# Shinokawa/Fast-SCNN-pytorch

Measured on AMD Instinct MI355X. Metric: images/sec fwd+bwd @1024x2048 bs=8 per GPU; 1/2/4/8-GPU scaling, higher is better.
Workload: dtype bf16; 1 GPU; cfg3 train step: fwd + CE(ignore -1) + bwd + fused SGD (fused low-res upsample+CE head); model=FastSCNN (19 classes), global_batch=8, per_gpu_batch=8, parallelism=dp1

## Files before the change

fast-scnn-pytorch_amd/_lib.py:

```python
import ctypes
import os
import threading

_HERE = os.path.dirname(os.path.abspath(__file__))
LIB_PATH = os.environ.get("FSCNN_LIB", os.path.join(_HERE, "libfastscnn_hip.so"))

DT_F32, DT_BF16, DT_F16 = 0, 1, 2
DT_U8 = 3

c_int, c_ll, c_float, c_vp, c_char_p = (ctypes.c_int, ctypes.c_longlong, ctypes.c_float,
                                        ctypes.c_void_p, ctypes.c_char_p)
c_ull, c_double = ctypes.c_ulonglong, ctypes.c_double
P_int, P_ll, P_vp = ctypes.POINTER(c_int), ctypes.POINTER(c_ll), ctypes.POINTER(c_vp)
P_float = ctypes.POINTER(c_float)
P_double = ctypes.POINTER(c_double)
c_uint, P_ubyte = ctypes.c_uint, ctypes.POINTER(ctypes.c_ubyte)


class AuxHead(ctypes.Structure):
    _fields_ = [("head", c_int), ("aux_weight", c_float), ("ignore_index", c_ll),
                ("smooth", c_float), ("dice_weight", c_float), ("focal_weight", c_float),
                ("alpha", c_float), ("gamma", c_float), ("thresh", c_float), ("min_kept", c_ll),
                ("class_weight", c_vp)]

# ... 110 lines not shown
                          c_int, c_float, c_vp]),
    "fscnn_adamw": (c_int, [c_vp, c_vp, c_vp, c_vp, c_vp, c_ll, c_double, c_double, c_double,
                            c_double, c_double, c_int, c_int, c_vp, c_int, c_vp, c_vp, c_vp]),
    "fscnn_adamw_segments": (c_int, [c_vp, c_vp, c_vp, c_vp, c_vp, c_vp, c_vp, c_int, c_vp, c_int,
                                     c_vp, c_int, c_vp, c_int, c_int, c_vp, c_vp, c_vp]),
    "fscnn_conv0_fwd": (c_int, [c_vp, c_int, c_int, c_int, c_int, c_vp, c_vp, c_vp, c_int, c_vp,
                                c_int, c_vp]),
    "fscnn_conv0_wgrad_slab_floats": (c_ll, [c_int, c_int, c_int]),
    "fscnn_conv0_wgrad": (c_int, [c_vp, c_int, c_int, c_int, c_int, c_vp, c_int, c_vp, c_vp, c_vp]),
    "fscnn_dw3x3_fwd": (c_int, [c_vp, c_int, c_int, c_int, c_int, c_int, c_int, c_vp, c_vp, c_vp,
                                c_int, c_vp, c_vp]),
    "fscnn_dw3x3_dgrad": (c_int, [c_vp, c_int, c_int, c_int, c_int, c_int, c_int, c_vp, c_vp,
                                  c_vp]),
    "fscnn_dw3x3_wgrad_slab_floats": (c_ll, [c_int, c_int, c_int, c_int, c_int, c_int]),
    "fscnn_dw3x3_wgrad": (c_int, [c_vp, c_vp, c_int, c_int, c_int, c_int, c_int, c_int, c_vp,
                                  c_vp, c_vp]),
    "fscnn_pw_gemm": (c_int, [c_int, c_int, c_int, c_vp, c_int, c_vp, c_int, c_int, c_vp, c_vp,
                              c_vp, c_int, c_int, c_vp, c_int, c_vp, c_int, c_vp]),
    "fscnn_pw_dgrad_bnbwd": (c_int, [c_int, c_int, c_int, c_vp, c_int, c_vp, c_int, c_vp, c_int,
                                     c_vp, c_int, c_vp, c_int, c_vp, c_vp, c_vp, c_vp, c_int,
                                     c_vp, c_vp, c_vp, c_vp, c_vp, c_vp, c_int, P_int, c_vp]),
    "fscnn_kth_smallest": (c_int, [c_vp, c_ll, c_ll, c_vp, c_vp, c_vp]),
    "fscnn_debug_stamps": (c_int, [c_vp, c_int]),
    "fscnn_debug_stamp_count": (c_int, []),
    "fscnn_debug_stamp_tag": (c_char_p, [c_int]),
    "fscnn_pw_wgrad_slab_floats": (c_ll, [c_int, c_int, c_int]),
    "fscnn_pw_gemm_stats_parts": (c_int, [c_int, c_int, c_int, c_int, c_int, c_int]),
    "fscnn_pw_wgrad": (c_int, [c_int, c_int, c_int, c_vp, c_int, c_vp, c_int, c_vp, c_vp, c_int,
                               c_vp]),
    "fscnn_bn_finalize": (c_int, [c_vp, c_int, c_int, c_vp, c_vp, c_vp, c_vp, c_vp, c_float,
                                  c_vp, c_vp, c_vp, c_vp, c_vp]),
    "fscnn_bilinear_ac_fwd": (c_int, [c_vp, c_int, c_int, c_int, c_int, c_int, c_int, c_int,
                                      c_vp, c_int, c_int, c_vp]),
    "fscnn_bilinear_ac_bwd": (c_int, [c_vp, c_int, c_int, c_int, c_int, c_int, c_int, c_int,
                                      c_vp, c_vp, c_vp]),
    "fscnn_pyramid_pool_fwd": (c_int, [c_vp, c_int, c_int, c_int, c_int, c_int, c_int, c_vp,
                                       c_vp]),
    "fscnn_block_ir_fwd": (c_int, [c_vp, c_int, c_int, c_int, c_int, c_int, c_int, c_int, c_int,
                                   c_vp, c_vp, c_vp, c_vp, c_vp, c_vp, c_vp, c_vp, c_vp, c_int,
                                   c_vp, c_int, c_vp]),
    "fscnn_pyramid_pool_bwd": (c_int, [c_vp, c_int, c_int, c_int, c_int, c_int, c_vp, c_int,
                                       c_int, c_vp]),
    "fscnn_bn_apply": (c_int, [c_ll, c_int, c_vp, c_int, c_vp, c_vp, c_vp, c_int, c_vp, c_vp, c_vp,
                               c_int, c_int, c_vp, c_int, c_int, c_vp]),
    "fscnn_bn_bwd": (c_int, [c_ll, c_int, c_vp, c_int, c_vp, c_int, c_vp, c_vp, c_vp, c_vp, c_vp,
                             c_int, c_int, c_vp, c_vp, c_vp, c_vp, c_vp, c_vp, c_vp, c_vp, c_vp,
                             c_vp, c_vp, c_vp, c_vp, c_int, P_int, P_int, c_vp]),
    "fscnn_ppm_branches_ok": (c_int, [c_int, c_int, c_int]),
    "fscnn_ppm_branches_fwd": (c_int, [c_int, P_int, c_int, c_vp, c_vp, c_vp, c_vp, c_vp, c_vp,
                                       c_vp, c_float, c_vp, c_vp, c_int, c_vp, c_vp, c_vp, c_vp,
                                       c_int, c_vp]),
    "fscnn_ppm_branches_bwd": (c_int, [c_int, P_int, c_int, c_vp, c_int, c_vp, c_int, c_vp, c_vp,
                                       c_vp, c_vp, c_vp, c_vp, c_vp, c_vp, c_vp, c_vp, c_vp, c_int,
                                       c_vp]),
    "fscnn_ppm_up_fwd": (c_int, [c_vp, c_int, c_int, c_int, c_int, c_vp, c_int, c_int, c_vp]),
    "fscnn_ppm_up_bwd": (c_int, [c_vp, c_int, c_int, c_int, c_int, c_int, c_int, c_vp, c_vp]),
    "fscnn_dropout": (c_int, [c_vp, c_int, c_int, c_int, c_int, c_int, c_int, c_ull, c_vp, c_ull,
                              c_float, c_vp, c_vp, c_vp, c_int, c_vp]),
    "fscnn_dw3x3_parts": (c_int, [c_int, c_int, c_int, c_int, c_int, c_int, c_int]),
    "fscnn_dw3x3_ct_width": (c_int, [c_int, c_int, c_int, c_int, c_int, c_int]),
    "fscnn_dw3x3_fwd_train": (c_int, [c_vp, c_int, c_int, c_int, c_int, c_int, c_int, c_vp, c_vp,
                                      c_vp, c_vp, c_vp, c_vp, c_vp, c_vp, c_vp, c_vp, c_vp, c_vp,
                                      c_float, c_vp, c_vp, c_vp, c_vp, P_int, c_vp]),
    "fscnn_dw3x3_dgrad_bn": (c_int, [c_vp, c_int, c_int, c_int, c_int, c_int, c_int, c_vp, c_vp,
                                     c_vp, c_vp, c_vp, c_vp, c_vp, c_int, c_vp, c_vp, c_vp, c_vp,
                                     c_vp, c_vp, P_int, c_vp]),
    "fscnn_dw3x3_wgrad_train": (c_int, [c_vp, c_vp, c_int, c_int, c_int, c_int, c_int, c_int,
                                        c_vp, c_vp, c_vp, c_vp, c_vp]),
    "fscnn_pw_fwd_train_route": (c_int, [c_int, c_int, c_int, c_int, c_int, c_int, c_int, P_int]),
    "fscnn_pw_fwd_train": (c_int, [c_int, c_int, c_int, c_vp, c_int, c_vp, c_vp, c_vp, c_int, c_vp,
                                   c_vp, c_int, c_vp, c_vp, c_vp, c_vp, c_vp, c_vp, c_vp, c_vp,
                                   c_float, c_vp, c_vp, c_vp, c_vp, c_int, P_int, P_int, c_vp]),
    "fscnn_pw_wgrad_train": (c_int, [c_int, c_int, c_int, c_vp, c_int, c_vp, c_int, c_vp, c_vp,
                                     c_vp, c_vp, c_vp, c_vp, c_int, P_int, c_vp]),
    "fscnn_pw_dgrad_train_route": (c_int, [c_int, c_int, c_int, c_int, c_int, c_int, c_int, c_int,
                                           P_int]),
    "fscnn_pw_dgrad_train": (c_int, [c_int, c_int, c_int, c_vp, c_int, c_vp, c_int, c_vp, c_int,
                                     c_vp, c_int, c_vp, c_int, c_vp, c_vp, c_vp, c_vp, c_int,
                                     c_vp, c_vp, c_vp, c_vp, c_vp, c_vp, c_vp, c_int, c_float,
                                     c_ull, c_ull, c_vp, c_int, P_int, P_int, c_vp]),
    "fscnn_im2col3": (c_int, [c_vp, c_int, c_int, c_int, c_int, c_int, c_int, c_vp, c_int, c_vp]),
    "fscnn_col2im3": (c_int, [c_vp, c_int, c_int, c_int, c_int, c_int, c_int, c_vp, c_int, c_int,
                              c_vp]),
    "fscnn_block_ir_s2_fwd": (c_int, [c_vp, c_int, c_int, c_int, c_int, c_int, c_int, c_int, c_int,
                                      c_vp, c_vp, c_vp, c_vp, c_vp, c_vp, c_vp, c_vp, c_vp, c_vp,
                                      c_int, c_vp]),
    "fscnn_block_ltd_fwd": (c_int, [c_vp, c_int, c_int, c_int, c_int, c_int, c_vp, c_vp, c_vp,
                                    c_vp, c_vp, c_vp, c_vp, c_vp, c_vp, c_vp, c_int, c_vp]),
    "fscnn_block_dsconv_fwd": (c_int, [c_vp, c_int, c_int, c_int, c_int, c_int, c_int, c_vp, c_vp,
                                       c_vp, c_vp, c_vp, c_vp, c_vp, c_int, c_vp]),
    "fscnn_block_dsconv_res_fwd": (c_int, [c_vp, c_int, c_int, c_int, c_int, c_int, c_int, c_int,
                                           c_int, c_vp, c_vp, c_vp, c_vp, c_vp, c_vp, c_vp, c_int,
                                           c_vp, c_int, c_vp]),
    "fscnn_block_cls_fwd": (c_int, [c_vp, c_int, c_int, c_int, c_int] + [c_vp] * 14 + [c_int, c_vp, c_vp,
                                                                              c_int, c_vp]),
    "fscnn_block_ffm_fwd": (c_int, [c_vp, c_int, c_int, c_int, c_int, c_int, c_int, c_vp, c_int,
                                    c_vp, c_vp, c_vp, c_vp, c_vp, c_vp, c_vp, c_vp, c_vp, c_vp,
                                    c_int, c_vp]),
}

_lib = None
_lock = threading.Lock()


def load():
    global _lib
    if _lib is not None:
        return _lib
    with _lock:
        if _lib is not None:
            return _lib
        if not os.path.exists(LIB_PATH):
            raise RuntimeError(
                "libfastscnn_hip.so not found at %s — build it with "
                "`python -c 'import __graft_entry__; __graft_entry__.build()'` "
                "(there is no CPU fallback)" % LIB_PATH)
        import torch
        lib = ctypes.CDLL(LIB_PATH, mode=ctypes.RTLD_GLOBAL)
        for name, (res, args) in SIGNATURES.items():
            fn = getattr(lib, name)
            fn.restype = res
            fn.argtypes = args
        _lib = lib
        return lib


def check(rc, what=""):
    if rc != 0:
        msg = load().fscnn_last_error().decode(errors="replace")
        raise RuntimeError("fastscnn HIP error %d in %s: %s" % (rc, what, msg))


def call(name, *args):
    rc = getattr(load(), name)(*args)
    check(rc, name)
    return rc


def ptr(t):
    return None if t is None else c_vp(t.data_ptr())


def stream_ptr(device=None):
    import torch
    return c_vp(torch.cuda.current_stream(device).cuda_stream)


def dtype_code(dt):
    import torch
    if dt == torch.float32:
        return DT_F32
    if dt == torch.bfloat16:
        return DT_BF16
    if dt == torch.float16:
        return DT_F16
    raise RuntimeError("fastscnn: unsupported dtype %s (fp32 / bf16 / fp16)" % (dt,))
```

fast-scnn-pytorch_amd/csrc/capi.cpp:

```cpp
#include <algorithm>
#include <chrono>
#include <cmath>
#include <cstdlib>
#include <cstdarg>
#include <cstdio>
#include <cstring>
#include <new>
#include <string>

#include "../../include/fastscnn.h"
#include "net.hpp"

namespace fscnn {

static thread_local char g_err[512] = "";

void set_error(const char* fmt, ...) {
  va_list ap;
  va_start(ap, fmt);
  vsnprintf(g_err, sizeof g_err, fmt, ap);
  va_end(ap);
}
const char* last_error() { return g_err; }

// ... 1802 lines not shown
  g.tail.tab.scale = scale; g.tail.tab.shift = shift; g.tail.tab.mean = mean;
  g.tail.tab.invstd = invstd;
  g.tail.tab.relu = relu_mode == 2;
  if (drop_hw > 0) {
    g.drop_hw = drop_hw; g.drop_thr = dropout_threshold(drop_p); g.drop_p = drop_p;
    g.drop_seed = seed; g.drop_seed_ptr = reinterpret_cast<const uint64_t*>(seed_slot);
    g.drop_seed_add = seed_add;
  }
  return g;
}

static int pw_dgrad_train_check(int M, int N, int K, int ldd, int ldb, int ldr, int has_r,
                                int lddx, int ldz, int relu_mode, int drop_hw, float drop_p,
                                int dtype) {
  const int rc = pw_geom_check("fscnn_pw_dgrad_train", dtype, M, N, K, ldd, ldb, lddx);
  if (rc) return rc;
  const int V = vec_w(dtype);
  if ((relu_mode != 0 && relu_mode != 2) || N > 1024 || !ld_ok(ldz, N, V) ||
      (has_r && !ld_ok(ldr, N, V))) {
    set_error("fscnn_pw_dgrad_train: relu_mode %d N=%d ldz=%d ldr=%d (relu_mode 0 or 2, N <= 1024, "
              "ldz / ldr >= N and a multiple of %d)", relu_mode, N, ldz, ldr, V);
    return E_INVALID;
  }
  if (drop_hw < 0 || (drop_hw > 0 && (!(drop_p >= 0.f && drop_p < 1.f) || M % drop_hw))) {
    set_error("fscnn_pw_dgrad_train: dropout hw %d p %g (0 <= p < 1, M a multiple of hw)", drop_hw,
              (double)drop_p);
    return E_INVALID;
  }
  return OK;
}

static int pw_dgrad_drop_check(const GemmArgs& g, int dtype) {
  if (g.drop_hw && !gemm_stream_ok(g, dtype)) {
    set_error("fscnn_pw_dgrad_train: an output dropout needs the streaming kernel, which does "
              "not take M=%d N=%d K=%d in dtype %d", g.M, g.N, g.K, dtype);
    return E_UNSUPPORTED;
  }
  return OK;
}

int fscnn_pw_dgrad_train_route(int M, int N, int K, int ldd, int lddx, int residual, int drop_hw,
                               int dtype, int* records) {
  if (pw_dgrad_train_check(M, N, K, ldd, ldd, lddx, residual, lddx, lddx, 0, drop_hw, 0.1f, dtype))
    return -1;
  static float f;
  static unsigned u;
  static double d;
  const GemmArgs g = pw_dgrad_train_args(M, N, K, &f, ldd, &f, ldd, residual ? &f : nullptr, lddx,
                                         &f, lddx, &f, lddx, &f, &f, &f, &f, 0, &f, &u, &d, &f,
                                         &f, &f, &f, drop_hw, 0.1f, 0, 0, nullptr);
  if (pw_dgrad_drop_check(g, dtype)) return -1;
  return pw_route(g, dtype, records);
}

int fscnn_pw_dgrad_train(int M, int N, int K, const void* D, int ldd, const void* B, int ldb,
                         const void* R, int ldr, void* dX, int lddx, const void* z, int ldz,
                         const float* mean, const float* invstd, const float* scale,
                         const float* shift, int relu_mode, float* part, unsigned* counters,
                         double* tsum, float* dgamma, float* dbeta, float* coef, float* tab,
                         int drop_hw, float drop_p, unsigned long long seed,
                         unsigned long long seed_add, const unsigned long long* seed_slot,
                         int dtype, int* route, int* records, void* stream) {
  if (!D || !B || !dX || !z || !mean || !invstd || !scale || !shift || !part || !counters ||
      !tsum || !dgamma || !dbeta || !coef || !tab || (uintptr_t)tab % 16) {
    set_error("fscnn_pw_dgrad_train: null argument (or tab not 16-byte aligned)");
    return E_INVALID;
  }
  int rc = pw_dgrad_train_check(M, N, K, ldd, ldb, ldr, R != nullptr, lddx, ldz, relu_mode,
                                drop_hw, drop_p, dtype);
  if (rc) return rc;
  const GemmArgs g = pw_dgrad_train_args(M, N, K, D, ldd, B, ldb, R, ldr, dX, lddx, z, ldz, mean,
                                         invstd, scale, shift, relu_mode, part, counters, tsum,
                                         dgamma, dbeta, coef, tab, drop_hw, drop_p, seed, seed_add,
                                         seed_slot);
  rc = pw_dgrad_drop_check(g, dtype);
  if (rc) return rc;
  int P;
  const int rt = pw_route(g, dtype, &P);
  if (route) *route = rt;
  if (records) *records = P;
  return gemm_nt(g, dtype, S(stream));
}

static int col3_check(const char* who, int dtype, int N, int H, int W, int C, const void* x, int ldx,
                      const void* col, int ldcol) {
  if (!x || !col) {
    set_error("%s: null argument", who);
    return E_INVALID;
  }
  if (!dt_ok(dtype)) {
    set_error("%s: dtype %d", who, dtype);
    return E_INVALID;
  }
  if (N < 1 || H < 1 || W < 1 || C < 1 || ldx < C || ldcol < 9 * C) {
    set_error("%s: N=%d H=%d W=%d C=%d, row strides %d (>= C) and %d (>= 9 C)", who, N, H, W, C,
              ldx, ldcol);
    return E_INVALID;
  }
  return OK;
}

int fscnn_im2col3(const void* x, int ldx, int dtype, int N, int H, int W, int C, void* col,
                  int ldcol, void* stream) {
  const int rc = col3_check("fscnn_im2col3", dtype, N, H, W, C, x, ldx, col, ldcol);
  if (rc) return rc;
  Im2ColArgs a{};
  a.N = N; a.H = H; a.W = W; a.C = C; a.x = x; a.ldx = ldx; a.col = col; a.ldcol = ldcol;
  return im2col3(a, dtype, S(stream));
}

int fscnn_col2im3(const void* dcol, int ldcol, int dtype, int N, int H, int W, int C, void* dx,
                  int lddx, int accumulate, void* stream) {
  const int rc = col3_check("fscnn_col2im3", dtype, N, H, W, C, dx, lddx, dcol, ldcol);
  if (rc) return rc;
  Col2ImArgs a{};
  a.N = N; a.H = H; a.W = W; a.C = C; a.dcol = dcol; a.ldcol = ldcol; a.dx = dx; a.lddx = lddx;
  a.accumulate = accumulate != 0;
  return col2im3(a, dtype, S(stream));
}

int fscnn_block_ir_fwd(const void* x, int ldx, int dtype, int N, int H, int W, int cin, int expand,
                       int cout, const void* w_expand, const float* w_dw, const void* w_project,
                       const float* scale_e, const float* shift_e, const float* scale_d,
                       const float* shift_d, const float* scale_p, const float* shift_p,
                       int residual, void* y, int ldy, void* stream) {
  if (!x || !y || !w_expand || !w_dw || !w_project || !scale_e || !shift_e || !scale_d ||
      !shift_d || !scale_p || !shift_p) {
    set_error("fscnn_block_ir_fwd: null argument");
    return E_INVALID;
  }
  if (dtype < DT_F32 || dtype > DT_F16) {
    set_error("fscnn_block_ir_fwd: dtype %d", dtype);
    return E_INVALID;
  }
  IrArgs a{};
  a.N = N; a.H = H; a.W = W; a.Cin = cin; a.E = expand; a.Cout = cout;
  a.x = x; a.ldx = ldx; a.y = y; a.ldy = ldy;
  a.we = w_expand; a.wd = w_dw; a.wp = w_project;
  a.sc_e = scale_e; a.sh_e = shift_e; a.sc_d = scale_d; a.sh_d = shift_d;
  a.sc_p = scale_p; a.sh_p = shift_p; a.residual = residual;
  return ir_block_fwd(a, dtype, S(stream));
}

int fscnn_block_ir_s2_fwd(const void* x, int ldx, int dtype, int N, int H, int W, int cin,
                          int expand, int cout, const void* w_expand, const float* w_dw,
                          const void* w_project, const float* scale_e, const float* shift_e,
                          const float* scale_d, const float* shift_d, const float* scale_p,
                          const float* shift_p, void* y, int ldy, void* stream) {
  if (!x || !y || !w_expand || !w_dw || !w_project || !scale_e || !shift_e || !scale_d ||
      !shift_d || !scale_p || !shift_p) {
    set_error("fscnn_block_ir_s2_fwd: null argument");
    return E_INVALID;
  }
  if (dtype < DT_F32 || dtype > DT_F16 || H < 1 || W < 1) {
    set_error("fscnn_block_ir_s2_fwd: dtype %d H %d W %d", dtype, H, W);
    return E_INVALID;
  }
  IrArgs a{};
  a.stride = 2; a.Hi = H; a.Wi = W;
  a.N = N; a.H = (H - 1) / 2 + 1; a.W = (W - 1) / 2 + 1; a.Cin = cin; a.E = expand; a.Cout = cout;
  a.x = x; a.ldx = ldx; a.y = y; a.ldy = ldy;
  a.we = w_expand; a.wd = w_dw; a.wp = w_project;
  a.sc_e = scale_e; a.sh_e = shift_e; a.sc_d = scale_d; a.sh_d = shift_d;
  a.sc_p = scale_p; a.sh_p = shift_p; a.residual = 0;
  return ir_block_fwd(a, dtype, S(stream));
}
// ... 150 lines not shown
```

fast-scnn-pytorch_amd/csrc/conv0.hip:

```cpp
#include "bn_finish.hpp"

namespace fscnn {

constexpr int C0_OUT = 32;
constexpr int C0_TILE = 256;
constexpr int C0_IN_W = 2 * C0_TILE + 1;
constexpr int C0_OSTR = 36;



__device__ __forceinline__ void c0_tile(int& seg, int& row) {
  const int gx = gridDim.x;
  const long long T = (long long)gx * gridDim.y;
  long long L = blockIdx.x + (long long)gx * blockIdx.y;
  if ((T & 7) == 0) L = (L & 7) * (T >> 3) + (L >> 3);
  seg = (int)(L % gx);
  row = (int)(L / gx);
}

#ifndef C0_RB_DEFAULT
#define C0_RB_DEFAULT 1
#endif
constexpr int C0_RB = C0_RB_DEFAULT;

// ... 482 lines not shown
      else prof_launch(conv0_wgrad_kernel<T, 0>, P, 256, 0, st, a);                            \
    }                                                                                 \
  } while (0)
  if (dz_dtype == DT_F32) CW_LAUNCH(float);
  else if (dz_dtype == DT_F16) CW_LAUNCH(f16);
  else CW_LAUNCH(bf16);
#undef CW_LAUNCH
  return check_launch("conv0_wgrad");
}

template <typename T, typename TO>
__global__ __launch_bounds__(256) void conv0_dgrad_kernel(Conv0DgradArgs a) {
  constexpr int V = VecW<T>::V;
  __shared__ float sw[9][3][32];
  for (int i = threadIdx.x; i < 864; i += 256) {
    const int co = i / 27, r = i - co * 27, ci = r / 9, k = r - ci * 9;
    sw[k][ci][co] = a.w[i];
  }
  __syncthreads();
  const long long HW = (long long)a.H * a.W;
  const long long p = (long long)blockIdx.x * 256 + threadIdx.x;
  if (p >= (long long)a.N * HW) return;
  const int n = (int)(p / HW);
  const long long hw = p - (long long)n * HW;
  const int h = (int)(hw / a.W), w = (int)(hw - (long long)h * a.W);
  float acc[3] = {0.f, 0.f, 0.f};
#pragma unroll
  for (int dh = 0; dh < 2; ++dh) {
    const int kh = (h & 1) + 2 * dh;
    const int oh = (h - kh) >> 1;
    if (kh > 2 || oh < 0 || oh >= a.Ho) continue;
#pragma unroll
    for (int dw = 0; dw < 2; ++dw) {
      const int kw = (w & 1) + 2 * dw;
      const int ow = (w - kw) >> 1;
      if (kw > 2 || ow < 0 || ow >= a.Wo) continue;
      const T* d = (const T*)a.dz + (((size_t)n * a.Ho + oh) * a.Wo + ow) * 32;
      const int k = kh * 3 + kw;
#pragma unroll
      for (int q = 0; q < 32 / V; ++q) {
        float v[V];
        unpack<T>(*reinterpret_cast<const uint4*>(d + q * V), v);
#pragma unroll
        for (int j = 0; j < V; ++j) {
          const int co = q * V + j;
          acc[0] = fmaf(v[j], sw[k][0][co], acc[0]);
          acc[1] = fmaf(v[j], sw[k][1][co], acc[1]);
          acc[2] = fmaf(v[j], sw[k][2][co], acc[2]);
        }
      }
    }
  }
  TO* dx = (TO*)a.dx + (size_t)n * 3 * HW + hw;
#pragma unroll
  for (int ci = 0; ci < 3; ++ci) st1(dx + ci * HW, acc[ci]);
}

int conv0_dgrad(const Conv0DgradArgs& a, int dz_dtype, hipStream_t st) {
  if (!a.dz || !a.w || !a.dx || a.N < 1 || a.Ho != (a.H - 3) / 2 + 1 || a.Wo != (a.W - 3) / 2 + 1) {
    set_error("conv0_dgrad: bad arguments (N %d, %dx%d -> %dx%d)", a.N, a.H, a.W, a.Ho, a.Wo);
    return E_INVALID;
  }
  if ((uintptr_t)a.dz % 16) {
    set_error("conv0_dgrad: dz must be 16-B aligned");
    return E_INVALID;
  }
  const int blocks = cdiv((long long)a.N * a.H * a.W, 256);
#define C0D_LAUNCH(T)                                                                          \
  do {                                                                                         \
    if (a.dx_dtype == DT_BF16) prof_launch(conv0_dgrad_kernel<T, bf16>, blocks, 256, 0, st, a);         \
    else if (a.dx_dtype == DT_F16) prof_launch(conv0_dgrad_kernel<T, f16>, blocks, 256, 0, st, a);      \
    else prof_launch(conv0_dgrad_kernel<T, float>, blocks, 256, 0, st, a);                              \
  } while (0)
  if (dz_dtype == DT_F32) C0D_LAUNCH(float);
  else if (dz_dtype == DT_F16) C0D_LAUNCH(f16);
  else C0D_LAUNCH(bf16);
#undef C0D_LAUNCH
  return check_launch("conv0_dgrad");
}

constexpr int LC_TW = 128;
constexpr int LC_LDX = 256 + 8;
constexpr int LC_MAXP = 512;
typedef float f32x16 __attribute__((ext_vector_type(16)));

template <typename T>
__device__ __forceinline__ void lc_mma(const i16x8& a, const i16x8& b, f32x16& acc) {
  if constexpr (std::is_same<T, f16>::value) {
    h16x8 ah, bh;
    __builtin_memcpy(&ah, &a, 16);
    __builtin_memcpy(&bh, &b, 16);
    acc = __builtin_amdgcn_mfma_f32_32x32x16_f16(ah, bh, acc, 0, 0, 0);
  } else {
    acc = __builtin_amdgcn_mfma_f32_32x32x16_bf16(a, b, acc, 0, 0, 0);
  }
}
template <typename T>
__device__ __forceinline__ void lc_unpack4(const uint2& t, float (&v)[4]) {
  v[0] = s16_to<T>((uint16_t)(t.x & 0xFFFFu)); v[1] = s16_to<T>((uint16_t)(t.x >> 16));
  v[2] = s16_to<T>((uint16_t)(t.y & 0xFFFFu)); v[3] = s16_to<T>((uint16_t)(t.y >> 16));
}
template <typename T>
__device__ __forceinline__ uint2 lc_pack4(const float (&v)[4]) {
  uint2 t;
  t.x = (uint32_t)s16_from<T>(v[0]) | ((uint32_t)s16_from<T>(v[1]) << 16);
  t.y = (uint32_t)s16_from<T>(v[2]) | ((uint32_t)s16_from<T>(v[3]) << 16);
  return t;
}
__device__ __forceinline__ i16x4 lc_tr(const uint16_t* p) {
  return __builtin_amdgcn_ds_read_tr16_b64_v4i16((__attribute__((address_space(3))) i16x4*)p);
}

template <typename T, int XB>
__global__ __launch_bounds__(256, 2) void ltd_c0_bwd_kernel(LtdC0BwdArgs a) {
  constexpr int V = 4;
  constexpr int SG = 256 * 32 * 2;
  __shared__ __attribute__((aligned(16))) unsigned char s_raw[2 * SG + 32 * LC_LDX * 2];
  uint16_t* sG = reinterpret_cast<uint16_t*>(s_raw);
  uint16_t* sZ = reinterpret_cast<uint16_t*>(s_raw + SG);
  uint16_t* sX = reinterpret_cast<uint16_t*>(s_raw + 2 * SG);
  const int tid = threadIdx.x, lane = tid & 63, wave = tid >> 6;
  const int tx = tid & 7, ty = tid >> 3;
  const int cb = tx * V;
  for (int i = tid; i < 5 * LC_LDX; i += 256) sX[27 * LC_LDX + i] = 0;

  __shared__ __attribute__((aligned(16))) float s_wt[9 * 32];
  __shared__ __attribute__((aligned(16))) float s_bn[4 * 32];
  for (int i = tid; i < 9 * 32; i += 256) s_wt[(i % 9) * 32 + i / 9] = a.w[i];
  if (tid < 32) {
    const bool m2 = a.bs.mode == 2;
    s_bn[tid] = a.bs.mean[tid];
    s_bn[32 + tid] = a.bs.invstd[tid];
    s_bn[64 + tid] = m2 ? a.bs.scale[tid] : 0.f;
    s_bn[96 + tid] = m2 ? a.bs.shift[tid] : 1.f;
  }
  __syncthreads();
  float s1[V], s2[V];
#pragma unroll
  for (int j = 0; j < V; ++j) s1[j] = s2[j] = 0.f;
  float bx[3][3];
#pragma unroll
  for (int i = 0; i < 3; ++i)
#pragma unroll
    for (int k = 0; k < 3; ++k) bx[i][k] = 0.f;
  f32x16 accA, accZ;
#pragma unroll
  for (int r = 0; r < 16; ++r) accA[r] = accZ[r] = 0.f;

  const int CB = cdiv(a.W, LC_TW), RP = (a.H + 1) / 2;
  const int tiles = a.N * RP * CB;
  const size_t XHW = (size_t)a.XH * a.XW;
  const int t_end = (int)((long long)tiles * (blockIdx.x + 1) / gridDim.x);
  for (int t = (int)((long long)tiles * blockIdx.x / gridDim.x); t < t_end; ++t) {
    const int nc = t / RP, hp = t - nc * RP;
    const int n = nc / CB, cbk = nc - n * CB;
    const int h0 = 2 * hp, wc0 = cbk * LC_TW, w0 = wc0 + 4 * ty;
    uint2 gr[2][3], zr[2][4];
    const T* gb = (const T*)a.dy + (size_t)n * a.Ho * a.Wo * 32 + cb;
#pragma unroll
    for (int dr = 0; dr < 2; ++dr)
#pragma unroll
      for (int dc = 0; dc < 3; ++dc) {
        const int ho = hp + dr, wo = w0 / 2 + dc;
        const bool ok = ho < a.Ho && wo < a.Wo && w0 < a.W;
        const uint2 v = *reinterpret_cast<const uint2*>(gb + (ok ? ho * a.Wo + wo : 0) * 32);
        gr[dr][dc] = ok ? v : make_uint2(0u, 0u);
      }
#pragma unroll
    for (int r = 0; r < 2; ++r)
#pragma unroll
      for (int q = 0; q < 4; ++q) {
        const bool ok = h0 + r < a.H && w0 + q < a.W;
        const size_t pix = ok ? ((size_t)n * a.H + h0 + r) * a.W + w0 + q : 0;
        const uint2 v = *reinterpret_cast<const uint2*>((const T*)a.bs.z + pix * 32 + cb);
        zr[r][q] = ok ? v : make_uint2(0u, 0u);
      }
    uint4 xr[3][XB ? 1 : 2];
    float x8[3];
#pragma unroll
    for (int it = 0; it < 3; ++it) {
      const int i = tid + 256 * it;
      if (i >= 576) break;
      const int pair = i >> 6, r = (i >> 5) & 1, u = i & 31;
      const int ci = pair / 3, kh = pair - 3 * ci;
      const int h = h0 + r, wq = wc0 + 4 * u;
      const bool okr = h < a.H && wq < a.W;
      const int col = okr ? 2 * wq : 0;
      const size_t o = ((size_t)n * 3 + ci) * XHW + (size_t)(okr ? 2 * h + kh : 0) * a.XW + col;
      const bool ok8 = okr && col + 8 < a.XW;
      if constexpr (XB) {
        xr[it][0] = *reinterpret_cast<const uint4*>((const uint16_t*)a.x + o);
        const uint16_t e8 = ((const uint16_t*)a.x)[ok8 ? o + 8 : o];
        x8[it] = ok8 ? in16<XB>(e8) : 0.f;
      } else {
        xr[it][0] = *reinterpret_cast<const uint4*>((const float*)a.x + o);
        xr[it][1] = *reinterpret_cast<const uint4*>((const float*)a.x + o + 4);
        const float e8 = ((const float*)a.x)[ok8 ? o + 8 : o];
        x8[it] = ok8 ? e8 : 0.f;
      }
    }
    uint2 gw[2][4];
#pragma unroll
    for (int r = 0; r < 2; ++r) {
      float acc[4][V];
#pragma unroll
      for (int q = 0; q < 4; ++q)
#pragma unroll
        for (int j = 0; j < V; ++j) acc[q][j] = 0.f;
#pragma unroll
      for (int dr = 0; dr < 2; ++dr) {
        const int kh = r + 1 - 2 * dr;
        if (kh < 0 || kh > 2) continue;
#pragma unroll
        for (int dc = 0; dc < 3; ++dc) {
          float g[V];
          lc_unpack4<T>(gr[dr][dc], g);
#pragma unroll
          for (int q = 0; q < 4; ++q) {
            const int kw = q + 1 - 2 * dc;
            if (kw < 0 || kw > 2) continue;
            const float4 w4 = *reinterpret_cast<const float4*>(s_wt + (kh * 3 + kw) * 32 + cb);
            const float wv[4] = {w4.x, w4.y, w4.z, w4.w};
#pragma unroll
            for (int j = 0; j < V; ++j) acc[q][j] = fmaf(g[j], wv[j], acc[q][j]);
          }
        }
      }
      const float4 bm = *reinterpret_cast<const float4*>(s_bn + cb);
      const float4 bi = *reinterpret_cast<const float4*>(s_bn + 32 + cb);
      const float4 ms = *reinterpret_cast<const float4*>(s_bn + 64 + cb);
      const float4 mh = *reinterpret_cast<const float4*>(s_bn + 96 + cb);
      const float bmv[4] = {bm.x, bm.y, bm.z, bm.w}, biv[4] = {bi.x, bi.y, bi.z, bi.w};
      const float msv[4] = {ms.x, ms.y, ms.z, ms.w}, mhv[4] = {mh.x, mh.y, mh.z, mh.w};
#pragma unroll
      for (int q = 0; q < 4; ++q) {
        const bool ok = h0 + r < a.H && w0 + q < a.W;
        float z[V], gv[V], zc[V];
        lc_unpack4<T>(zr[r][q], z);
#pragma unroll
        for (int j = 0; j < V; ++j) {
          float v = round_as<T>(acc[q][j]);
          v = (ok && fmaf(z[j], msv[j], mhv[j]) > 0.f) ? v : 0.f;
          zc[j] = z[j] - bmv[j];
          s1[j] += v;
          s2[j] += v * zc[j] * biv[j];
          gv[j] = v;
        }
        gw[r][q] = lc_pack4<T>(gv);
        zr[r][q] = lc_pack4<T>(zc);
      }
    }
    uint2 xw[3][3];
#pragma unroll
    for (int it = 0; it < 3; ++it) {
      const int i = tid + 256 * it;
      if (i >= 576) break;
      const int r = (i >> 5) & 1, u = i & 31;
      const int h = h0 + r, wq = wc0 + 4 * u;
      float xe[9];
      if constexpr (XB) {
        const uint32_t wv[4] = {xr[it][0].x, xr[it][0].y, xr[it][0].z, xr[it][0].w};
#pragma unroll
        for (int k = 0; k < 4; ++k) {
          xe[2 * k] = in16<XB>((uint16_t)(wv[k] & 0xFFFFu));
          xe[2 * k + 1] = in16<XB>((uint16_t)(wv[k] >> 16));
        }
      } else {
#pragma unroll
        for (int k = 0; k < 2; ++k) {
          xe[4 * k] = __uint_as_float(xr[it][k].x); xe[4 * k + 1] = __uint_as_float(xr[it][k].y);
          xe[4 * k + 2] = __uint_as_float(xr[it][k].z); xe[4 * k + 3] = __uint_as_float(xr[it][k].w);
        }
      }
      xe[8] = x8[it];
#pragma unroll
      for (int kw = 0; kw < 3; ++kw) {
        float v[4];
#pragma unroll
        for (int q = 0; q < 4; ++q) {
          const bool ok = h < a.H && wq + q < a.W;
          v[q] = ok ? round_as<T>(xe[2 * q + kw]) : 0.f;
        }
        bx[it][kw] += (v[0] + v[1]) + (v[2] + v[3]);
        xw[it][kw] = lc_pack4<T>(v);
      }
    }
    __syncthreads();
#pragma unroll
    for (int r = 0; r < 2; ++r)
#pragma unroll
      for (int q = 0; q < 4; ++q) {
        const int p = r * 128 + 4 * ty + q;
        *reinterpret_cast<uint2*>(sG + p * 32 + cb) = gw[r][q];
        *reinterpret_cast<uint2*>(sZ + p * 32 + cb) = zr[r][q];
      }
#pragma unroll
    for (int it = 0; it < 3; ++it) {
      const int i = tid + 256 * it;
      if (i >= 576) break;
      const int pair = i >> 6, r = (i >> 5) & 1, u = i & 31;
#pragma unroll
      for (int kw = 0; kw < 3; ++kw)
        *reinterpret_cast<uint2*>(sX + (pair * 3 + kw) * LC_LDX + r * 128 + 4 * u) = xw[it][kw];
    }
    __syncthreads();
    {
      const int g4 = lane >> 4, li = lane & 15;
      const int rq = 8 * (g4 >> 1) + (li >> 2), cc = 16 * (g4 & 1) + 4 * (li & 3);
#pragma unroll
      for (int ks = 0; ks < 4; ++ks) {
        const int k0 = wave * 64 + ks * 16;
        i16x8 ax;
        __builtin_memcpy(&ax, sX + (lane & 31) * LC_LDX + k0 + 8 * (lane >> 5), 16);
        const uint16_t* pg = sG + (k0 + rq) * 32 + cc;
        const uint16_t* pz = sZ + (k0 + rq) * 32 + cc;
        const i16x4 g0 = lc_tr(pg), g1 = lc_tr(pg + 4 * 32);
        const i16x4 z0 = lc_tr(pz), z1 = lc_tr(pz + 4 * 32);
        const i16x8 bg = {g0[0], g0[1], g0[2], g0[3], g1[0], g1[1], g1[2], g1[3]};
        const i16x8 bz = {z0[0], z0[1], z0[2], z0[3], z1[0], z1[1], z1[2], z1[3]};
        lc_mma<T>(ax, bg, accA);
        lc_mma<T>(ax, bz, accZ);
      }
    }
  }

  __syncthreads();
  float* red = reinterpret_cast<float*>(s_raw);
#pragma unroll
  for (int r = 0; r < 16; ++r) {
    const int m = (r & 3) + 8 * (r >> 2) + 4 * (lane >> 5);
    red[((wave * 2 + 0) * 32 + m) * 32 + (lane & 31)] = accA[r];
    red[((wave * 2 + 1) * 32 + m) * 32 + (lane & 31)] = accZ[r];
  }
  __syncthreads();
  float* out = a.slab + (size_t)blockIdx.x * LC0_SLAB;
  for (int o = tid; o < 1728; o += 256) {
    const int k = o >= 864 ? 1 : 0, oo = o - 864 * k;
    const int co = oo / 27, tap = oo - 27 * co;
    const int e = (k * 32 + tap) * 32 + co;
    out[o] = (red[e] + red[2048 + e]) + (red[4096 + e] + red[6144 + e]);
  }
#pragma unroll
  for (int it = 0; it < 3; ++it) {
    if (wave + 4 * it >= 9) break;
#pragma unroll
    for (int kw = 0; kw < 3; ++kw) {
      float v = bx[it][kw];
#pragma unroll
      for (int off = 32; off >= 1; off >>= 1) v += __shfl_xor(v, off);
      if (lane == 0) out[1728 + (wave + 4 * it) * 3 + kw] = v;
    }
  }
  float* s_br = reinterpret_cast<float*>(s_raw + 2 * SG);
#pragma unroll
  for (int j = 0; j < V; ++j) {
    s_br[tid * 2 * V + j] = s1[j];
    s_br[tid * 2 * V + V + j] = s2[j];
  }
  __syncthreads();
  if (tid < 64) {
    const int kind = tid >> 5, c = tid & 31;
    const int qx = c >> 2, j = c & 3;
    float sum = 0.f;
    for (int y = 0; y < 32; ++y) sum += s_br[(y * 8 + qx) * 2 * V + kind * V + j];
    a.bs.part[(size_t)blockIdx.x * 64 + kind * 32 + c] = sum;
  }
}

int ltd_c0_bwd_parts(int N, int H, int W) {
  const long long tiles = (long long)N * ((H + 1) / 2) * cdiv(W, LC_TW);
  return (int)(tiles < LC_MAXP ? tiles : LC_MAXP);
}

bool ltd_c0_bwd_ok(int dtype, int x_dtype, int XW, const void* x) {
  return (dtype == DT_BF16 || dtype == DT_F16) && x_dtype >= 0 && x_dtype <= 2 && XW % 8 == 0 &&
         (uintptr_t)x % 16 == 0;
}

int ltd_c0_bwd(const LtdC0BwdArgs& a, int dtype, hipStream_t st) {
  if (!ltd_c0_bwd_ok(dtype, a.x_dtype, a.XW, a.x) || a.H != (a.XH - 3) / 2 + 1 ||
      a.W != (a.XW - 3) / 2 + 1 || a.Ho != (a.H - 1) / 2 + 1 || a.Wo != (a.W - 1) / 2 + 1) {
    set_error("ltd_c0_bwd: unsupported shape / dtype / alignment");
    return E_INVALID;
  }
  if (!a.bs.part || !a.bs.z || !a.bs.mean || !a.bs.invstd ||
      (a.bs.mode == 2 && (!a.bs.scale || !a.bs.shift)) || !a.slab || (uintptr_t)a.w % 16 ||
      (uintptr_t)a.dy % 8 || (uintptr_t)a.bs.z % 8) {
    set_error("ltd_c0_bwd: inconsistent arguments");
    return E_INVALID;
  }
  if ((long long)a.N * ((a.H + 1) / 2) * cdiv(a.W, LC_TW) > 0x7fffffffLL ||
      (long long)a.Ho * a.Wo > 0x7fffffffLL / 32) {
    set_error("ltd_c0_bwd: tensor too large");
    return E_INVALID;
  }
  const int P = ltd_c0_bwd_parts(a.N, a.H, a.W);
  const bool fin = a.tail.counters != nullptr;
  {
    const double px = (double)a.N * a.H * a.W;
    ProfScope ps(PK_CONV0_WGRAD, st,
                 2.0 * ((double)a.N * a.Ho * a.Wo * 32 + px * 32) +
                     (a.x_dtype ? 2.0 : 4.0) * a.N * 3.0 * a.XH * a.XW + 36.0 * 32,
                 18.0 * (double)a.N * a.Ho * a.Wo * 32 + 4.0 * 27 * 32 * px);
#define LC_LAUNCH(T, XB) prof_launch(ltd_c0_bwd_kernel<T, XB>, P, 256, 0, st, a)
#define LC_LAUNCH_X(T)                            \
  do {                                            \
// ... 33 lines not shown
```

include/fastscnn.h:

```cpp
#ifndef FASTSCNN_H
#define FASTSCNN_H

#ifdef __cplusplus
extern "C" {
#endif

typedef struct fscnn_net fscnn_net;
typedef struct fscnn_plan fscnn_plan;

const char* fscnn_version(void);
const char* fscnn_last_error(void);

int fscnn_net_create(int num_classes, int aux, fscnn_net** out);
void fscnn_net_destroy(fscnn_net* net);
int fscnn_net_param_count(const fscnn_net* net, int* count, long long* total_floats);
int fscnn_net_param_info(const fscnn_net* net, int i, const char** name, long long* offset,
                         long long* numel);
int fscnn_net_buffer_count(const fscnn_net* net, int* count, long long* total_floats, int* num_bn);
int fscnn_net_buffer_info(const fscnn_net* net, int i, const char** name, long long* offset,
                          long long* numel);
int fscnn_net_stage_range(const fscnn_net* net, int stage, long long* begin, long long* end);

int fscnn_plan_create(const fscnn_net* net, int N, int H, int W, int dtype, int train,
                      fscnn_plan** out);
// ... 295 lines not shown
                      float* rmean, float* rvar, long long* nbt, float momentum, float* mean,
                      float* invstd, float* scale, float* shift, void* stream);
int fscnn_bilinear_ac_fwd(const void* x, int dtype, int N, int Hi, int Wi, int C, int Ho, int Wo,
                          void* y, int out_nchw, int out_dtype, void* stream);
int fscnn_bilinear_ac_bwd(const void* dy, int dtype, int N, int Hi, int Wi, int C, int Ho, int Wo,
                          float* tmp, void* dx, void* stream);
int fscnn_pyramid_pool_fwd(const void* x, int dtype, int N, int H, int W, int C, int ldx,
                           void* pooled, void* stream);
int fscnn_pyramid_pool_bwd(const void* dpooled, int dtype, int N, int H, int W, int C, void* dx,
                           int lddx, int accumulate, void* stream);

int fscnn_bn_apply(long long M, int C, const void* z, int ldz, const float* scale,
                   const float* shift, const void* z2, int ldz2, const float* scale2,
                   const float* shift2, const void* res, int ldres, int relu, void* y, int ldy,
                   int dtype, void* stream);
int fscnn_bn_bwd(long long M, int C, const void* dy, int lddy, const void* mask, int ldmask,
                 const void* z, const float* mean, const float* invstd, const float* scale,
                 const float* shift, int relu_mode, int frozen, const void* z2,
                 const float* mean2, const float* invstd2, const float* scale2, float* part,
                 unsigned* counters, void* dz, void* dz2, float* dgamma, float* dbeta,
                 float* dgamma2, float* dbeta2, float* coef, int dtype, int* P,
                 int* rows_per_block, void* stream);
int fscnn_ppm_branches_ok(int maxM, int K, int dtype);
int fscnn_ppm_branches_fwd(int nb, const int* M, int K, const void* x, const void* w,
                           const float* gamma, const float* beta, float* rmean, float* rvar,
                           long long* nbt, float momentum, void* z, void* y, int ldy, float* mean,
                           float* invstd, float* scale, float* shift, int dtype, void* stream);
int fscnn_ppm_branches_bwd(int nb, const int* M, int K, const void* dy, int lddy, const void* y,
                           int ldy, const void* z, const float* mean, const float* invstd,
                           const float* scale, const float* gamma, const void* x, const void* w,
                           float* dgamma, float* dbeta, float* dw, void* dx, int dtype,
                           void* stream);
int fscnn_ppm_up_fwd(const void* feats, int dtype, int N, int H, int W, void* y, int ldy, int coff,
                     void* stream);
int fscnn_ppm_up_bwd(const void* dy, int dtype, int N, int H, int W, int ldy, int coff,
                     void* dfeats, void* stream);
int fscnn_dropout(const void* x, int ldx, int dtype, int N, int H, int W, int C,
                  unsigned long long seed, const unsigned long long* seed_slot,
                  unsigned long long seed_add, float p, const float* x_scale,
                  const float* x_shift, void* y, int ldy, void* stream);
int fscnn_dw3x3_parts(int N, int H, int W, int C, int stride, int dtype, int dgrad);
int fscnn_dw3x3_ct_width(int N, int H, int W, int C, int stride, int dtype);
int fscnn_dw3x3_fwd_train(const void* x, int dtype, int N, int H, int W, int C, int stride,
                          const float* w, const float* in_scale, const float* in_shift, void* z,
                          float* part, unsigned* counters, double* tsum, const float* gamma,
                          const float* beta, float* rmean, float* rvar, long long* nbt,
                          float momentum, float* mean, float* invstd, float* scale, float* shift,
                          int* in_kernel, void* stream);
int fscnn_dw3x3_dgrad_bn(const void* dy, int dtype, int N, int H, int W, int C, int stride,
                         const float* w, void* dx, const void* z, const float* mean,
                         const float* invstd, const float* scale, const float* shift,
                         int relu_mode, float* part, unsigned* counters, double* tsum,
                         float* dgamma, float* dbeta, float* coef, int* in_kernel, void* stream);
int fscnn_dw3x3_wgrad_train(const void* x, const void* dy, int dtype, int N, int H, int W, int C,
                            int stride, const float* x_scale, const float* x_shift, float* slab,
                            float* dw, void* stream);

int fscnn_pw_fwd_train_route(int M, int N, int K, int lda, int ldc, int lazy, int dtype,
                             int* records);
int fscnn_pw_fwd_train(int M, int N, int K, const void* A, int lda, const float* a_scale,
                       const float* a_shift, const void* B, int ldb, const float* bias, void* z,
                       int ldc, float* part, unsigned* counters, double* tsum, const float* gamma,
                       const float* beta, float* rmean, float* rvar, long long* nbt,
                       float momentum, float* mean, float* invstd, float* scale, float* shift,
                       int dtype, int* route, int* records, void* stream);
int fscnn_pw_wgrad_train(int M, int N, int K, const void* D, int ldd, const void* X, int ldx,
                         const float* x_scale, const float* x_shift, float* slab, float* dW,
                         float* bias_part, float* dbias, int dtype, int* splits, void* stream);
int fscnn_pw_dgrad_train_route(int M, int N, int K, int ldd, int lddx, int residual, int drop_hw,
                               int dtype, int* records);
int fscnn_pw_dgrad_train(int M, int N, int K, const void* D, int ldd, const void* B, int ldb,
                         const void* R, int ldr, void* dX, int lddx, const void* z, int ldz,
                         const float* mean, const float* invstd, const float* scale,
                         const float* shift, int relu_mode, float* part, unsigned* counters,
                         double* tsum, float* dgamma, float* dbeta, float* coef, float* tab,
                         int drop_hw, float drop_p, unsigned long long seed,
                         unsigned long long seed_add, const unsigned long long* seed_slot,
                         int dtype, int* route, int* records, void* stream);
int fscnn_im2col3(const void* x, int ldx, int dtype, int N, int H, int W, int C, void* col,
                  int ldcol, void* stream);
int fscnn_col2im3(const void* dcol, int ldcol, int dtype, int N, int H, int W, int C, void* dx,
                  int lddx, int accumulate, void* stream);

#ifdef __cplusplus
}
#endif
#endif
```

Baseline: 1506 images/s.

## Prefetch next tile's global loads in fused LTD conv0 backward kernel

Restructures the persistent tile loop of the fused learning-to-downsample conv0 backward kernel so the global loads of dy, z and the input image for the next tile are issued before the current tile is staged into LDS and fed to MFMA. Staging now writes directly to shared memory instead of going through intermediate register arrays, and sched_barrier fences are added. Boundary masking moves from load time to consume time. The aim is to hide global-memory latency behind compute, at the cost of higher register pressure from holding two tiles' worth of loads. It also exposes a standalone C API entry point for the kernel, useful for testing.

```diff
diff --git a/fast-scnn-pytorch_amd/_lib.py b/fast-scnn-pytorch_amd/_lib.py
--- a/fast-scnn-pytorch_amd/_lib.py
+++ b/fast-scnn-pytorch_amd/_lib.py
@@ -216,6 +216,8 @@
     "fscnn_im2col3": (c_int, [c_vp, c_int, c_int, c_int, c_int, c_int, c_int, c_vp, c_int, c_vp]),
     "fscnn_col2im3": (c_int, [c_vp, c_int, c_int, c_int, c_int, c_int, c_int, c_vp, c_int, c_int,
                               c_vp]),
+    "fscnn_ltd_c0_bwd_parts": (c_int, [c_int, c_int, c_int]),
+    "fscnn_ltd_c0_bwd": (c_int, [c_vp] * 8 + [c_int] * 4 + [c_vp] * 10 + [c_int, c_vp]),
     "fscnn_block_ir_s2_fwd": (c_int, [c_vp, c_int, c_int, c_int, c_int, c_int, c_int, c_int, c_int,
                                       c_vp, c_vp, c_vp, c_vp, c_vp, c_vp, c_vp, c_vp, c_vp, c_vp,
                                       c_int, c_vp]),
diff --git a/fast-scnn-pytorch_amd/csrc/capi.cpp b/fast-scnn-pytorch_amd/csrc/capi.cpp
--- a/fast-scnn-pytorch_amd/csrc/capi.cpp
+++ b/fast-scnn-pytorch_amd/csrc/capi.cpp
@@ -1908,6 +1908,51 @@
   return gemm_nt(g, dtype, S(stream));
 }
 
+int fscnn_ltd_c0_bwd_parts(int N, int XH, int XW) {
+  if (N < 1 || XH < 3 || XW < 3) return 0;
+  return ltd_c0_bwd_parts(N, (XH - 3) / 2 + 1, (XW - 3) / 2 + 1);
+}
+
+int fscnn_ltd_c0_bwd(const void* dy, const void* z, const float* w_dw, const float* mean,
+                     const float* invstd, const float* scale, const float* shift, const void* x,
+                     int x_dtype, int N, int XH, int XW, float* part, unsigned* counters,
+                     double* tsum, float* dgamma, float* dbeta, float* coef, float* tab,
+                     float* slab, float* sums, float* dw, int dtype, void* stream) {
+  if (!dy || !z || !w_dw || !mean || !invstd || !scale || !shift || !x || !part || !counters ||
+      !tsum || !dgamma || !dbeta || !coef || !tab || (uintptr_t)tab % 16 || !slab || !sums) {
+    set_error("fscnn_ltd_c0_bwd: null argument (or tab not 16-byte aligned)");
+    return E_INVALID;
+  }
+  if (N < 1 || XH < 3 || XW < 3) {
+    set_error("fscnn_ltd_c0_bwd: N=%d image %dx%d", N, XH, XW);
+    return E_INVALID;
+  }
+  LtdC0BwdArgs f{};
+  f.N = N; f.H = (XH - 3) / 2 + 1; f.W = (XW - 3) / 2 + 1;
+  f.Ho = (f.H - 1) / 2 + 1; f.Wo = (f.W - 1) / 2 + 1;
+  f.dy = dy; f.w = w_dw;
+  f.bs.part = part;
+  f.bs.z = z;
+  f.bs.mean = mean; f.bs.invstd = invstd; f.bs.scale = scale; f.bs.shift = shift;
+  f.bs.mode = 2;
+  f.tail.counters = counters;
+  f.tail.tsum = tsum;
+  f.tail.count = (double)N * f.H * f.W;
+  f.tail.dgamma = dgamma; f.tail.dbeta = dbeta; f.tail.coef = coef;
+  f.tail.tab.tab = tab;
+  f.tail.tab.scale = scale; f.tail.tab.shift = shift; f.tail.tab.mean = mean;
+  f.tail.tab.invstd = invstd;
+  f.tail.tab.relu = true;
+  f.x = x; f.x_dtype = x_dtype; f.XH = XH; f.XW = XW;
+  f.slab = slab;
+  hipStream_t st = S(stream);
+  int rc = ltd_c0_bwd(f, dtype, st);
+  if (rc) return rc;
+  rc = reduce_slabs(slab, ltd_c0_bwd_parts(N, f.H, f.W), LC0_SLAB, LC0_SLAB, sums, 0, st);
+  if (rc || !dw) return rc;
+  return conv0_wgrad_combine(sums, tab, mean, dw, st);
+}
+
 static int col3_check(const char* who, int dtype, int N, int H, int W, int C, const void* x, int ldx,
                       const void* col, int ldcol) {
   if (!x || !col) {
diff --git a/fast-scnn-pytorch_amd/csrc/conv0.hip b/fast-scnn-pytorch_amd/csrc/conv0.hip
--- a/fast-scnn-pytorch_amd/csrc/conv0.hip
+++ b/fast-scnn-pytorch_amd/csrc/conv0.hip
@@ -588,6 +588,10 @@
 constexpr int LC_TW = 128;
 constexpr int LC_LDX = 256 + 8;
 constexpr int LC_MAXP = 512;
+#ifndef LC_PREFETCH
+#define LC_PREFETCH 1
+#endif
+#define LC_SCHED_FENCE() __builtin_amdgcn_sched_barrier(0)
 typedef float f32x16 __attribute__((ext_vector_type(16)));
 
 template <typename T>
@@ -656,33 +660,40 @@
   const int CB = cdiv(a.W, LC_TW), RP = (a.H + 1) / 2;
   const int tiles = a.N * RP * CB;
   const size_t XHW = (size_t)a.XH * a.XW;
-  const int t_end = (int)((long long)tiles * (blockIdx.x + 1) / gridDim.x);
-  for (int t = (int)((long long)tiles * blockIdx.x / gridDim.x); t < t_end; ++t) {
-    const int nc = t / RP, hp = t - nc * RP;
-    const int n = nc / CB, cbk = nc - n * CB;
-    const int h0 = 2 * hp, wc0 = cbk * LC_TW, w0 = wc0 + 4 * ty;
+  struct Tile {
+    int n, hp, cbk;
     uint2 gr[2][3], zr[2][4];
-    const T* gb = (const T*)a.dy + (size_t)n * a.Ho * a.Wo * 32 + cb;
+    uint4 xr[3][XB ? 1 : 2];
+    uint32_t x8[3];
+  };
+  auto tile_pos = [&](int t, Tile& L) {
+    const int nc = t / RP;
+    L.hp = t - nc * RP;
+    L.n = nc / CB;
+    L.cbk = nc - L.n * CB;
+  };
+  auto load_gz = [&](Tile& L) {
+    const int h0 = 2 * L.hp, w0 = L.cbk * LC_TW + 4 * ty;
+    const T* gb = (const T*)a.dy + (size_t)L.n * a.Ho * a.Wo * 32 + cb;
 #pragma unroll
     for (int dr = 0; dr < 2; ++dr)
 #pragma unroll
       for (int dc = 0; dc < 3; ++dc) {
-        const int ho = hp + dr, wo = w0 / 2 + dc;
+        const int ho = L.hp + dr, wo = w0 / 2 + dc;
         const bool ok = ho < a.Ho && wo < a.Wo && w0 < a.W;
-        const uint2 v = *reinterpret_cast<const uint2*>(gb + (ok ? ho * a.Wo + wo : 0) * 32);
-        gr[dr][dc] = ok ? v : make_uint2(0u, 0u);
+        L.gr[dr][dc] = *reinterpret_cast<const uint2*>(gb + (ok ? ho * a.Wo + wo : 0) * 32);
       }
 #pragma unroll
     for (int r = 0; r < 2; ++r)
 #pragma unroll
       for (int q = 0; q < 4; ++q) {
         const bool ok = h0 + r < a.H && w0 + q < a.W;
-        const size_t pix = ok ? ((size_t)n * a.H + h0 + r) * a.W + w0 + q : 0;
-        const uint2 v = *reinterpret_cast<const uint2*>((const T*)a.bs.z + pix * 32 + cb);
-        zr[r][q] = ok ? v : make_uint2(0u, 0u);
-      }
-    uint4 xr[3][XB ? 1 : 2];
-    float x8[3];
+        const size_t pix = ok ? ((size_t)L.n * a.H + h0 + r) * a.W + w0 + q : 0;
+        L.zr[r][q] = *reinterpret_cast<const uint2*>((const T*)a.bs.z + pix * 32 + cb);
+      }
+  };
+  auto load_x = [&](Tile& L) {
+    const int h0 = 2 * L.hp, wc0 = L.cbk * LC_TW;
 #pragma unroll
     for (int it = 0; it < 3; ++it) {
       const int i = tid + 256 * it;
@@ -692,20 +703,57 @@
       const int h = h0 + r, wq = wc0 + 4 * u;
       const bool okr = h < a.H && wq < a.W;
       const int col = okr ? 2 * wq : 0;
-      const size_t o = ((size_t)n * 3 + ci) * XHW + (size_t)(okr ? 2 * h + kh : 0) * a.XW + col;
+      const size_t o = ((size_t)L.n * 3 + ci) * XHW + (size_t)(okr ? 2 * h + kh : 0) * a.XW + col;
       const bool ok8 = okr && col + 8 < a.XW;
       if constexpr (XB) {
-        xr[it][0] = *reinterpret_cast<const uint4*>((const uint16_t*)a.x + o);
-        const uint16_t e8 = ((const uint16_t*)a.x)[ok8 ? o + 8 : o];
-        x8[it] = ok8 ? in16<XB>(e8) : 0.f;
+        L.xr[it][0] = *reinterpret_cast<const uint4*>((const uint16_t*)a.x + o);
+        L.x8[it] = *reinterpret_cast<const uint32_t*>((const uint16_t*)a.x + (ok8 ? o + 8 : o));
       } else {
-        xr[it][0] = *reinterpret_cast<const uint4*>((const float*)a.x + o);
-        xr[it][1] = *reinterpret_cast<const uint4*>((const float*)a.x + o + 4);
-        const float e8 = ((const float*)a.x)[ok8 ? o + 8 : o];
-        x8[it] = ok8 ? e8 : 0.f;
-      }
-    }
-    uint2 gw[2][4];
+        L.xr[it][0] = *reinterpret_cast<const uint4*>((const float*)a.x + o);
+        L.xr[it][1] = *reinterpret_cast<const uint4*>((const float*)a.x + o + 4);
+        L.x8[it] = ((const uint32_t*)a.x)[ok8 ? o + 8 : o];
+      }
+    }
+  };
+  auto stage = [&](Tile& L) {
+    const int h0 = 2 * L.hp, wc0 = L.cbk * LC_TW, w0 = wc0 + 4 * ty;
+#pragma unroll
+    for (int it = 0; it < 3; ++it) {
+      const int i = tid + 256 * it;
+      if (i >= 576) break;
+      const int pair = i >> 6, r = (i >> 5) & 1, u = i & 31;
+      const int h = h0 + r, wq = wc0 + 4 * u;
+      const bool ok8 = h < a.H && wq < a.W && 2 * wq + 8 < a.XW;
+      float xe[9];
+      if constexpr (XB) {
+        const uint32_t wv[4] = {L.xr[it][0].x, L.xr[it][0].y, L.xr[it][0].z, L.xr[it][0].w};
+#pragma unroll
+        for (int k = 0; k < 4; ++k) {
+          xe[2 * k] = in16<XB>((uint16_t)(wv[k] & 0xFFFFu));
+          xe[2 * k + 1] = in16<XB>((uint16_t)(wv[k] >> 16));
+        }
+        xe[8] = ok8 ? in16<XB>((uint16_t)L.x8[it]) : 0.f;
+      } else {
+#pragma unroll
+        for (int k = 0; k < 2; ++k) {
+          xe[4 * k] = __uint_as_float(L.xr[it][k].x); xe[4 * k + 1] = __uint_as_float(L.xr[it][k].y);
+          xe[4 * k + 2] = __uint_as_float(L.xr[it][k].z); xe[4 * k + 3] = __uint_as_float(L.xr[it][k].w);
+        }
+        xe[8] = ok8 ? __uint_as_float(L.x8[it]) : 0.f;
+      }
+#pragma unroll
+      for (int kw = 0; kw < 3; ++kw) {
+        float v[4];
+#pragma unroll
+        for (int q = 0; q < 4; ++q) {
+          const bool ok = h < a.H && wq + q < a.W;
+          v[q] = ok ? round_as<T>(xe[2 * q + kw]) : 0.f;
+        }
+        bx[it][kw] += (v[0] + v[1]) + (v[2] + v[3]);
+        *reinterpret_cast<uint2*>(sX + (pair * 3 + kw) * LC_LDX + r * 128 + 4 * u) = lc_pack4<T>(v);
+      }
+      LC_SCHED_FENCE();
+    }
 #pragma unroll
     for (int r = 0; r < 2; ++r) {
       float acc[4][V];
@@ -719,8 +767,9 @@
         if (kh < 0 || kh > 2) continue;
 #pragma unroll
         for (int dc = 0; dc < 3; ++dc) {
+          const bool okg = L.hp + dr < a.Ho && w0 / 2 + dc < a.Wo && w0 < a.W;
           float g[V];
-          lc_unpack4<T>(gr[dr][dc], g);
+          lc_unpack4<T>(okg ? L.gr[dr][dc] : make_uint2(0u, 0u), g);
 #pragma unroll
           for (int q = 0; q < 4; ++q) {
             const int kw = q + 1 - 2 * dc;
@@ -742,7 +791,7 @@
       for (int q = 0; q < 4; ++q) {
         const bool ok = h0 + r < a.H && w0 + q < a.W;
         float z[V], gv[V], zc[V];
-        lc_unpack4<T>(zr[r][q], z);
+        lc_unpack4<T>(ok ? L.zr[r][q] : make_uint2(0u, 0u), z);
 #pragma unroll
         for (int j = 0; j < V; ++j) {
           float v = round_as<T>(acc[q][j]);
@@ -752,82 +801,59 @@
           s2[j] += v * zc[j] * biv[j];
           gv[j] = v;
         }
-        gw[r][q] = lc_pack4<T>(gv);
-        zr[r][q] = lc_pack4<T>(zc);
-      }
-    }
-    uint2 xw[3][3];
-#pragma unroll
-    for (int it = 0; it < 3; ++it) {
-      const int i = tid + 256 * it;
-      if (i >= 576) break;
-      const int r = (i >> 5) & 1, u = i & 31;
-      const int h = h0 + r, wq = wc0 + 4 * u;
-      float xe[9];
-      if constexpr (XB) {
-        const uint32_t wv[4] = {xr[it][0].x, xr[it][0].y, xr[it][0].z, xr[it][0].w};
-#pragma unroll
-        for (int k = 0; k < 4; ++k) {
-          xe[2 * k] = in16<XB>((uint16_t)(wv[k] & 0xFFFFu));
-          xe[2 * k + 1] = in16<XB>((uint16_t)(wv[k] >> 16));
-        }
-      } else {
-#pragma unroll
-        for (int k = 0; k < 2; ++k) {
-          xe[4 * k] = __uint_as_float(xr[it][k].x); xe[4 * k + 1] = __uint_as_float(xr[it][k].y);
-          xe[4 * k + 2] = __uint_as_float(xr[it][k].z); xe[4 * k + 3] = __uint_as_float(xr[it][k].w);
-        }
-      }
-      xe[8] = x8[it];
-#pragma unroll
-      for (int kw = 0; kw < 3; ++kw) {
-        float v[4];
-#pragma unroll
-        for (int q = 0; q < 4; ++q) {
-          const bool ok = h < a.H && wq + q < a.W;
-          v[q] = ok ? round_as<T>(xe[2 * q + kw]) : 0.f;
-        }
-        bx[it][kw] += (v[0] + v[1]) + (v[2] + v[3]);
-        xw[it][kw] = lc_pack4<T>(v);
-      }
-    }
+        const int p = r * 128 + 4 * ty + q;
+        *reinterpret_cast<uint2*>(sG + p * 32 + cb) = lc_pack4<T>(gv);
+        *reinterpret_cast<uint2*>(sZ + p * 32 + cb) = lc_pack4<T>(zc);
+      }
+      LC_SCHED_FENCE();
+    }
+  };
+  auto mfma = [&]() {
+    const int g4 = lane >> 4, li = lane & 15;
+    const int rq = 8 * (g4 >> 1) + (li >> 2), cc = 16 * (g4 & 1) + 4 * (li & 3);
+#pragma unroll
+    for (int ks = 0; ks < 4; ++ks) {
+      const int k0 = wave * 64 + ks * 16;
+      i16x8 ax;
+      __builtin_memcpy(&ax, sX + (lane & 31) * LC_LDX + k0 + 8 * (lane >> 5), 16);
+      const uint16_t* pg = sG + (k0 + rq) * 32 + cc;
+      const uint16_t* pz = sZ + (k0 + rq) * 32 + cc;
+      const i16x4 g0 = lc_tr(pg), g1 = lc_tr(pg + 4 * 32);
+      const i16x4 z0 = lc_tr(pz), z1 = lc_tr(pz + 4 * 32);
+      const i16x8 bg = {g0[0], g0[1], g0[2], g0[3], g1[0], g1[1], g1[2], g1[3]};
+      const i16x8 bz = {z0[0], z0[1], z0[2], z0[3], z1[0], z1[1], z1[2], z1[3]};
+      lc_mma<T>(ax, bg, accA);
+      lc_mma<T>(ax, bz, accZ);
+    }
+  };
+  constexpr bool PF = LC_PREFETCH != 0;
+  const int t_end = (int)((long long)tiles * (blockIdx.x + 1) / gridDim.x);
+  const int t_beg = (int)((long long)tiles * blockIdx.x / gridDim.x);
+  Tile nxt = {};
+  if (PF && t_beg < t_end) {
+    tile_pos(t_beg, nxt);
+    load_gz(nxt);
+    load_x(nxt);
+    __builtin_amdgcn_s_waitcnt(0x0F70);
+  }
+  for (int t = t_beg; t < t_end; ++t) {
+    Tile cur = nxt;
+    nxt = Tile{};
+    if (!PF) {
+      tile_pos(t, cur);
+      load_gz(cur);
+      load_x(cur);
+    } else if (t + 1 < t_end) {
+      tile_pos(t + 1, nxt);
+      load_gz(nxt);
+      load_x(nxt);
+    }
+    LC_SCHED_FENCE();
     __syncthreads();
-#pragma unroll
-    for (int r = 0; r < 2; ++r)
-#pragma unroll
-      for (int q = 0; q < 4; ++q) {
-        const int p = r * 128 + 4 * ty + q;
-        *reinterpret_cast<uint2*>(sG + p * 32 + cb) = gw[r][q];
-        *reinterpret_cast<uint2*>(sZ + p * 32 + cb) = zr[r][q];
-      }
-#pragma unroll
-    for (int it = 0; it < 3; ++it) {
-      const int i = tid + 256 * it;
-      if (i >= 576) break;
-      const int pair = i >> 6, r = (i >> 5) & 1, u = i & 31;
-#pragma unroll
-      for (int kw = 0; kw < 3; ++kw)
-        *reinterpret_cast<uint2*>(sX + (pair * 3 + kw) * LC_LDX + r * 128 + 4 * u) = xw[it][kw];
-    }
+    stage(cur);
+    LC_SCHED_FENCE();
     __syncthreads();
-    {
-      const int g4 = lane >> 4, li = lane & 15;
-      const int rq = 8 * (g4 >> 1) + (li >> 2), cc = 16 * (g4 & 1) + 4 * (li & 3);
-#pragma unroll
-      for (int ks = 0; ks < 4; ++ks) {
-        const int k0 = wave * 64 + ks * 16;
-        i16x8 ax;
-        __builtin_memcpy(&ax, sX + (lane & 31) * LC_LDX + k0 + 8 * (lane >> 5), 16);
-        const uint16_t* pg = sG + (k0 + rq) * 32 + cc;
-        const uint16_t* pz = sZ + (k0 + rq) * 32 + cc;
-        const i16x4 g0 = lc_tr(pg), g1 = lc_tr(pg + 4 * 32);
-        const i16x4 z0 = lc_tr(pz), z1 = lc_tr(pz + 4 * 32);
-        const i16x8 bg = {g0[0], g0[1], g0[2], g0[3], g1[0], g1[1], g1[2], g1[3]};
-        const i16x8 bz = {z0[0], z0[1], z0[2], z0[3], z1[0], z1[1], z1[2], z1[3]};
-        lc_mma<T>(ax, bg, accA);
-        lc_mma<T>(ax, bz, accZ);
-      }
-    }
+    mfma();
   }
 
   __syncthreads();
diff --git a/include/fastscnn.h b/include/fastscnn.h
--- a/include/fastscnn.h
+++ b/include/fastscnn.h
@@ -401,6 +401,13 @@
 int fscnn_col2im3(const void* dcol, int ldcol, int dtype, int N, int H, int W, int C, void* dx,
                   int lddx, int accumulate, void* stream);
 
+int fscnn_ltd_c0_bwd_parts(int N, int XH, int XW);
+int fscnn_ltd_c0_bwd(const void* dy, const void* z, const float* w_dw, const float* mean,
+                     const float* invstd, const float* scale, const float* shift, const void* x,
+                     int x_dtype, int N, int XH, int XW, float* part, unsigned* counters,
+                     double* tsum, float* dgamma, float* dbeta, float* coef, float* tab,
+                     float* slab, float* sums, float* dw, int dtype, void* stream);
+
 #ifdef __cplusplus
 }
 #endif
```

Result: no change. 1513 images/s (median of 6 runs) (+0.5%).
